# kimerein/sabatinilab-glm

Measured on AMD Instinct MI355X. Metric: IRLS iters/sec on 1M×2000 design mat; CV-grid wall-clock (5-fold×20 λ), lower is better.
Workload: dtype bf16 Hessian (w rounded to bf16, X exact 0/1) / exact-f32 gradient (3 bf16 pieces, f64 slab sums) / f64 coefficients and line search

## Files before the change

sabatinilab-glm_amd/csrc/chol.hip:

```cpp
#include <cstdlib>
#include <cstring>
#include <functional>
#include <map>
#include <mutex>
#include <vector>

#include "common.h"
#include "chol_tile.h"

namespace sglm {

constexpr int kNB = 64;
constexpr int kCT = 256;
constexpr int kMaxP = 8192;

void launch_chol_diag(int nact, hipStream_t s, float* Hall, int32_t P, int32_t k0,
                      const int32_t* fits, uint8_t* frozen_all, float* rhs_all,
                      const float* diag_all, int32_t* info, int32_t nrefac, float* minv_all,
                      float* Mall);
void launch_chol_diag4(int nact, hipStream_t s, float* Hall, int32_t P, int32_t k0,
                       const int32_t* fits, uint8_t* frozen_all, const float* diag_all,
                       int32_t* info, float* minv_all, float* Mall);

void launch_chol_diag4q(int nact, hipStream_t s, float* Hall, int32_t P, int32_t k0,
                        const int32_t* fits, uint8_t* frozen_all, const float* diag_all,
                        int32_t* info, float* minv_all, float* Mall);
void launch_chol_diag4l(int nact, hipStream_t s, float* Hall, int32_t P, int32_t k0,
                        const int32_t* fits, uint8_t* frozen_all, const float* diag_all,
                        int32_t* info, float* minv_all, float* Mall);
void launch_chol_update_diag4l(dim3 grid, hipStream_t s, float* Hall, int32_t P, int32_t k0,
                               int32_t kc, int32_t s0, const int32_t* fits, uint8_t* frozen_all,
                               const float* diag_all, int32_t* info, float* minv_all,
                               float* Mall);

static bool diag4q() {
    const char* e = getenv("SGLM_DIAG4Q");
    return !(e && e[0] == '0');
}

static bool diag4l() {
    const char* e = getenv("SGLM_DIAG4L");
    return !(e && e[0] == '0');
}

static bool upd_diag() {
    const char* e = getenv("SGLM_UPD_DIAG");
    return !(e && e[0] == '0');
}

static bool diag4() {
    static const bool v = [] {
        const char* e = getenv("SGLM_DIAG4");
        return !(e && e[0] == '0');
    }();
    return v;
}


__global__ void __launch_bounds__(kCT) chol_prep_kernel(
    float* __restrict__ Hall, int32_t P, const int32_t* __restrict__ fits,
    const double* __restrict__ gall, const float* __restrict__ dshift_all,
    uint8_t* __restrict__ frozen_all, float* __restrict__ rhs_all, float* __restrict__ diag_all,
    int32_t* __restrict__ info, int32_t nrefac) {
    const int fit = fits[blockIdx.x];
    const bool refactor = (int)blockIdx.x < nrefac;
    float* H = Hall + (int64_t)fit * P * P;
    const float* dsh = dshift_all + (int64_t)fit * P;
    uint8_t* frz = frozen_all + (int64_t)fit * P;
    float* rhs = rhs_all + (int64_t)fit * P;
    float* dg = diag_all + (int64_t)fit * P;
    const int tid = threadIdx.x;
    if (refactor) {
        if (tid == 0) info[fit] = 0;
        for (int j = tid; j < P; j += kCT) {
            const float d = H[(int64_t)j * P + j] + dsh[j];
            const bool f = dsh[j] < 0.0f || !(d > 0.0f);
            frz[j] = f;
            dg[j] = f ? 1.0f : d;
            H[(int64_t)j * P + j] = f ? 1.0f : d;
        }
    }
    if (!gall) return;
    const double* g = gall + (int64_t)fit * P;
    __syncthreads();
    for (int j = tid; j < P; j += kCT) rhs[j] = frz[j] ? 0.0f : (float)g[j];
}

__global__ void __launch_bounds__(kCT) chol_freeze_kernel(float* __restrict__ Hall, int32_t P,
                                                          const int32_t* __restrict__ fits,
                                                          const uint8_t* __restrict__ frozen_all) {
    const int fit = fits[blockIdx.y];
    float* H = Hall + (int64_t)fit * P * P;
    const uint8_t* frz = frozen_all + (int64_t)fit * P;
    int t = blockIdx.x, bi = 0;
    {
        int rowlen = P / kNB;
        while (t >= rowlen) { t -= rowlen; ++bi; --rowlen; }
    }
    const int bj = bi + t;
    __shared__ uint8_t fr[kNB], fc[kNB];
    __shared__ int any;
    const int tid = threadIdx.x;
    if (tid == 0) any = 0;
    __syncthreads();
    if (tid < kNB) {
        fr[tid] = frz[bi * kNB + tid];
        if (fr[tid]) any = 1;
    } else if (tid < 2 * kNB) {
        fc[tid - kNB] = frz[bj * kNB + tid - kNB];
        if (fc[tid - kNB]) any = 1;
    }
    __syncthreads();
    if (!any) return;
    const int c = tid & 63;
    for (int r = tid >> 6; r < kNB; r += kCT / 64) {
        const int i = bi * kNB + r, j = bj * kNB + c;
        if (i > j || !(fr[r] | fc[c])) continue;
        H[(int64_t)i * P + j] = i == j ? 1.0f : 0.0f;
    }
}

__global__ void __launch_bounds__(kCT) chol_alias_prep_kernel(
    int32_t P, const int32_t* __restrict__ fits, const int32_t* __restrict__ fsrc,
    const double* __restrict__ gall, const float* __restrict__ rscale,
    const uint8_t* __restrict__ frozen_all, float* __restrict__ rhs_all) {
    const int fit = fits[blockIdx.x];
    const uint8_t* frz = frozen_all + (int64_t)fsrc[blockIdx.x] * P;
    const double* g = gall + (int64_t)fit * P;
    float* rhs = rhs_all + (int64_t)fit * P;
    const double sc = (double)rscale[blockIdx.x];
    for (int j = threadIdx.x; j < P; j += kCT) rhs[j] = frz[j] ? 0.0f : (float)(g[j] * sc);
}

__device__ __forceinline__ float lanef(float v, int l) {
    return __int_as_float(__builtin_amdgcn_readlane(__float_as_int(v), l));
}

__global__ void __launch_bounds__(kCT) chol_panel_kernel(
    float* __restrict__ Hall, int32_t P, int32_t k0, const int32_t* __restrict__ fits,
    const float* __restrict__ minv_all, float* __restrict__ rhs_all, int32_t nrefac) {
    __shared__ float zs[kNB];
    __shared__ float sred[2][kNB];
    const int slot = blockIdx.x;
    const int fit = fits[slot];
    const bool refactor = slot < nrefac;
    float* H = Hall + (int64_t)fit * P * P;
    float* rhs = rhs_all + (int64_t)fit * P;
    const int tid = threadIdx.x, lane = tid & 63, wave = tid >> 6;
    const int r32 = lane & 31, kh = lane >> 5;
    const int rh = wave >> 1, ch = wave & 1;
    const int j0 = k0 + kNB + blockIdx.y * kNB;
    const int j = j0 + ch * 32 + r32;
    if (tid < kNB) zs[tid] = rhs[k0 + tid];
    float b[32];
    const float* pb = H + (int64_t)(k0 + kh) * P + j;
#pragma unroll
    for (int u = 0; u < 32; ++u) b[u] = pb[(int64_t)(2 * u) * P];
    __syncthreads();
    float s = 0.0f;
    if (refactor) {
        const float* pm = minv_all + (int64_t)slot * kNB * kNB + (rh * 32 + r32) * kNB + kh;
        float m[32];
#pragma unroll
        for (int u = 0; u < 32; ++u) m[u] = (rh || u < 16) ? pm[2 * u] : 0.0f;
        f32x16 acc = {};
#pragma unroll
        for (int u = 0; u < 16; ++u)
            acc = __builtin_amdgcn_mfma_f32_32x32x2f32(m[u], b[u], acc, 0, 0, 0);
        if (rh) {
#pragma unroll
            for (int u = 16; u < 32; ++u)
                acc = __builtin_amdgcn_mfma_f32_32x32x2f32(m[u], b[u], acc, 0, 0, 0);
        }
        __syncthreads();
#pragma unroll
        for (int q = 0; q < 16; ++q) {
            const int i = rh * 32 + (q & 3) + 8 * (q >> 2) + 4 * kh;
            H[(int64_t)(k0 + i) * P + j] = acc[q];
            s = fmaf(acc[q], zs[i], s);
        }
    } else if (rh == 0) {
#pragma unroll
        for (int u = 0; u < 32; ++u) s = fmaf(b[u], zs[2 * u + kh], s);
    }
    s += __shfl_xor(s, 32, 64);
    if (kh == 0) sred[rh][ch * 32 + r32] = s;
// ... 673 lines not shown
            for (int u = 0; u < 4; ++u) {
                float b[2];
#pragma unroll
                for (int qj = 0; qj < 2; ++qj)
                    b[qj] = sb[cur][(4 * kh + 8 * kk + u) * kLB2 + wc * 64 + qj * 32 + r32];
#pragma unroll
                for (int qi = 0; qi < 2; ++qi)
#pragma unroll
                    for (int qj = 0; qj < 2; ++qj)
                        acc[qi][qj] = __builtin_amdgcn_mfma_f32_32x32x2f32(a[qi][u], b[qj],
                                                                           acc[qi][qj], 0, 0, 0);
            }
        }
        if (more) sstore(cur ^ 1);
        __syncthreads();
        cur ^= 1;
    }
#pragma unroll
    for (int qi = 0; qi < 2; ++qi)
#pragma unroll
        for (int qj = 0; qj < 2; ++qj) {
            const int i0 = ti * kT2 + wr * 64 + qi * 32, j0 = tj * kT2 + wc * 64 + qj * 32;
#pragma unroll
            for (int q = 0; q < 16; ++q) {
                const int i = i0 + (q & 3) + 8 * (q >> 2) + 4 * kh, j = j0 + r32;
                if (STEP == 0)
                    T[(int64_t)i * s + j] = acc[qi][qj][q];
                else
                    M[(int64_t)(a0 + i) * P + c0 + j] = -acc[qi][qj][q];
            }
        }
}

template <bool SECOND, bool STAGE = false>
__global__ void __launch_bounds__(kCT) chol_inv_apply_kernel(
    const float* __restrict__ Mall, int32_t P, const int32_t* __restrict__ fits,
    const int32_t* __restrict__ fsrc, const float* __restrict__ rscale,
    const int32_t* __restrict__ tiles, const double* __restrict__ gall,
    const uint8_t* __restrict__ frozen_all, float* __restrict__ Y, float* __restrict__ delta_all) {
    __shared__ float red[4][16 * 64];
    __shared__ __attribute__((aligned(16))) float sm[STAGE ? 4 : 1][STAGE ? 64 * 32 : 4];
    const int start = tiles[2 * blockIdx.y], cnt = tiles[2 * blockIdx.y + 1];
    const int src = fsrc[start];
    const float* M = Mall + (int64_t)src * P * P;
    const uint8_t* frz = frozen_all + (int64_t)src * P;
    const int lane = threadIdx.x & 63, wave = threadIdx.x >> 6;
    const int r32 = lane & 31, kh = lane >> 5;
    const int c0 = blockIdx.x * 32;
    const bool valid = r32 < cnt;
    const int q = start + (valid ? r32 : 0);
    f32x16 acc = {};
    if (!SECOND) {
        const double* g = gall + (int64_t)fits[q] * P;
        const double sc = (double)rscale[q];
        const float* pb = M + c0 + r32;
        const int khi = (c0 / kNB + 1) * kNB;
        for (int kb = kNB * wave; kb < khi; kb += 4 * kNB) {
            float a[8][4], b[8][4];
            const float* pbk = pb + (int64_t)(kb + 4 * kh) * P;
            if (STAGE) {
                const float* src = M + (int64_t)kb * P + c0 + 4 * (lane & 7);
                f32x4 tv[8];
#pragma unroll
                for (int i = 0; i < 8; ++i)
                    tv[i] = *reinterpret_cast<const f32x4*>(src + (int64_t)((lane >> 3) + 8 * i) * P);
#pragma unroll
                for (int i = 0; i < 8; ++i)
                    *reinterpret_cast<f32x4*>(&sm[wave][((lane >> 3) + 8 * i) * 32 + 4 * (lane & 7)]) =
                        tv[i];
                asm volatile("s_waitcnt lgkmcnt(0)" ::: "memory");
                __builtin_amdgcn_wave_barrier();
            }
#pragma unroll
            for (int v = 0; v < 8; ++v) {
                const int k = kb + 8 * v + 4 * kh;
                const uint32_t fz = *reinterpret_cast<const uint32_t*>(frz + k);
                const double2 g01 = *reinterpret_cast<const double2*>(g + k);
                const double2 g23 = *reinterpret_cast<const double2*>(g + k + 2);
                a[v][0] = (float)(g01.x * sc);
                a[v][1] = (float)(g01.y * sc);
                a[v][2] = (float)(g23.x * sc);
                a[v][3] = (float)(g23.y * sc);
                const uint32_t keep = valid ? ~fz : 0u;
#pragma unroll
                for (int u = 0; u < 4; ++u) {
                    if (((keep >> (8 * u)) & 0xff) != 0xff) a[v][u] = 0.0f;
                    b[v][u] = STAGE ? sm[wave][(8 * v + 4 * kh + u) * 32 + r32]
                                    : pbk[(8 * v + u) * P];
                }
            }
#pragma unroll
            for (int v = 0; v < 8; ++v)
#pragma unroll
                for (int u = 0; u < 4; ++u)
                    acc = __builtin_amdgcn_mfma_f32_32x32x2f32(a[v][u], b[v][u], acc, 0, 0, 0);
            if (STAGE) {
                asm volatile("s_waitcnt lgkmcnt(0)" ::: "memory");
                __builtin_amdgcn_wave_barrier();
            }
        }
    } else {
        const float* py = Y + (int64_t)q * P;
        const float* pm = M + (int64_t)(c0 + r32) * P;
        const int klo = (c0 / kNB) * kNB;
        for (int kb = klo + kNB * wave; kb < P; kb += 4 * kNB) {
            f32x4 a[8], b[8];
#pragma unroll
            for (int v = 0; v < 8; ++v) {
                const int k = kb + 8 * v + 4 * kh;
                a[v] = *reinterpret_cast<const f32x4*>(py + k);
                if (!valid) a[v] = f32x4{0.0f, 0.0f, 0.0f, 0.0f};
                b[v] = *reinterpret_cast<const f32x4*>(pm + k);
            }
#pragma unroll
            for (int v = 0; v < 8; ++v)
#pragma unroll
                for (int u = 0; u < 4; ++u)
                    acc = __builtin_amdgcn_mfma_f32_32x32x2f32(a[v][u], b[v][u], acc, 0, 0, 0);
        }
    }
#pragma unroll
    for (int r = 0; r < 16; ++r) red[wave][r * 64 + lane] = acc[r];
    __syncthreads();
#pragma unroll
    for (int m = 0; m < 4; ++m) {
        const int o = threadIdx.x + kCT * m;
        const float v = red[0][o] + red[1][o] + red[2][o] + red[3][o];
        const int r = o >> 6, l = o & 63;
        const int row = (r & 3) + 8 * (r >> 2) + 4 * (l >> 5), col = c0 + (l & 31);
        if (row >= cnt) continue;
        if (!SECOND)
            Y[(int64_t)(start + row) * P + col] = v;
        else
            delta_all[(int64_t)fits[start + row] * P + col] = frz[col] ? 0.0f : -v;
    }
}

}

using namespace sglm;

static int64_t inv_tcap(int32_t P) {
    int64_t cap = 0;
    for (int s = kNB; s < P; s *= 2) {
        const int64_t pairs = (P - s + 2 * s - 1) / (2 * s);
        const int64_t v = pairs * s * s;
        cap = v > cap ? v : cap;
    }
    return cap;
}

extern "C" size_t sglm_chol_work_bytes(int32_t P, int32_t B) {
    return ((size_t)3 * (size_t)B * (size_t)P + (size_t)B * kNB * kNB +
            (size_t)B * (size_t)inv_tcap(P)) * sizeof(float);
}

static int chol_lookahead() {
    const char* e = getenv("SGLM_CHOL_LOOKAHEAD");
    const int v = e ? atoi(e) : 4;
    return v >= 1 && v <= 8 ? v : 4;
}

static bool inv_pipe() {
    static const bool v = [] {
        const char* e = getenv("SGLM_CHOL_PIPE");
        return !(e && e[0] == '0');
    }();
    return v;
}

static bool inv_x3() {
    const char* e = getenv("SGLM_INV_X3");
    return !(e && e[0] == '0');
}

static bool inv_lds() {
    static const bool v = [] {
        const char* e = getenv("SGLM_INV_LDS");
        return !(e && e[0] == '0');
    }();
    return v;
}

static bool inv128(int64_t wgs) {
    const char* e = getenv("SGLM_INV128_WG");
    const int64_t mn = e ? atoll(e) : 0;
    return mn > 0 && wgs >= mn;
}

static bool upd_pipe() {
    static const bool v = [] {
        const char* e = getenv("SGLM_UPD_PIPE");
        return e && e[0] == '1';
    }();
    return v;
}

static bool apply_stage() {
    static const bool v = [] {
        const char* e = getenv("SGLM_APPLY_STAGE");
        return !(e && e[0] == '0');
    }();
    return v;
}

static bool upd_lds() {
    static const bool v = [] {
        const char* e = getenv("SGLM_UPD_LDS");
        return !(e && e[0] == '0');
    }();
    return v;
}

static void launch_update(dim3 grid, hipStream_t s, float* H, int32_t P, int32_t k0, int32_t kc,
                          int32_t s0, const int32_t* fits) {
    if (upd_lds())
        chol_update_lds_kernel<<<grid, kCT, 0, s>>>(H, P, k0, kc, s0, fits);
    else if (upd_pipe())
        chol_update_kernel<true><<<grid, kCT, 0, s>>>(H, P, k0, kc, s0, fits);
    else
        chol_update_kernel<false><<<grid, kCT, 0, s>>>(H, P, k0, kc, s0, fits);
}

static int chol_solve_mixed(float* H, int32_t P, const int32_t* fits, int32_t nact,
                            int32_t nrefac, const double* g, const float* dshift, float* delta,
                            int32_t* info, uint8_t* frozen, int32_t B, void* work,
                            hipStream_t s, float* Mall = nullptr,
                            const std::function<void(int)>* on_diag = nullptr) {
    if (nact <= 0) return SGLM_OK;
    if (!H || !fits || (!g && !Mall) || !dshift || !delta || !info || !frozen || !work ||
        P % kNB || P > kMaxP || B < nact || nrefac < 0 || nrefac > nact) {
        set_error("sglm_chol_solve: bad args (P=%d, max %d)", P, kMaxP);
        return SGLM_EINVAL;
    }
    float* rhs = (float*)work;
    float* dg = rhs + (size_t)B * P;
    float* minv = dg + (size_t)B * P;
    chol_prep_kernel<<<nact, kCT, 0, s>>>(H, P, fits, g, dshift, frozen, rhs, dg, info, nrefac);
    int st = check_launch("chol_prep_kernel");
    if (st) return st;
    if (nrefac > 0) {
        const int nb = P / kNB;
        chol_freeze_kernel<<<dim3((unsigned)(nb * (nb + 1) / 2), (unsigned)nrefac), kCT, 0, s>>>(
            H, P, fits, frozen);
        if ((st = check_launch("chol_freeze_kernel"))) return st;
    }
    if (nrefac == 0 && Mall) return SGLM_OK;
    if (nrefac == 0) {
        chol_fwd2_kernel<<<nact, kST, 0, s>>>(H, P, fits, nullptr, frozen, rhs);
        st = check_launch("chol_fwd2_kernel");
        if (st) return st;
        chol_back2_kernel<<<nact, kST, 0, s>>>(H, P, fits, nullptr, frozen, rhs, delta);
        return check_launch("chol_back2_kernel");
    }
    const int nb = P / kNB;
    const bool fuse = Mall && nrefac == nact && diag4() && diag4q() && diag4l() && upd_lds() &&
                      upd_diag();
    bool have_diag = false;
    auto factor_step = [&](int kb) {
        const int k0 = kb * kNB;
        if (have_diag)
            ;
        else if (Mall && nrefac == nact && diag4() && diag4q() && diag4l())
            launch_chol_diag4l(nact, s, H, P, k0, fits, frozen, dg, info, minv, Mall);
        else if (Mall && nrefac == nact && diag4() && diag4q())
            launch_chol_diag4q(nact, s, H, P, k0, fits, frozen, dg, info, minv, Mall);
        else if (Mall && nrefac == nact && diag4())
            launch_chol_diag4(nact, s, H, P, k0, fits, frozen, dg, info, minv, Mall);
        else
            launch_chol_diag(nact, s, H, P, k0, fits, frozen, rhs, dg, info, nrefac, minv, Mall);
        if (!have_diag && on_diag) (*on_diag)(kb);
        const int rem = P - k0 - kNB;
        if (rem > 0)
            chol_panel_kernel<<<dim3(nact, rem / kNB), kCT, 0, s>>>(H, P, k0, fits, minv, rhs,
                                                                    nrefac);
    };
    const int la = chol_lookahead();
    for (int kb = 0; kb < nb; kb += la) {
        const int ke = kb + la < nb ? kb + la : nb;
        for (int b = kb; b < ke; ++b) {
            factor_step(b);
            have_diag = false;
            const int nr = ke - 1 - b;
            const int T = nb - b - 1;
            if (nrefac > 0 && nr > 0) {
                const dim3 g(nr * T - nr * (nr - 1) / 2, nrefac);
                if (fuse) {
                    launch_chol_update_diag4l(g, s, H, P, b * kNB, kNB, b + 1, fits, frozen, dg,
                                              info, minv, Mall);
                    have_diag = true;
                    if (on_diag) (*on_diag)(b + 1);
                } else {
                    launch_update(g, s, H, P, b * kNB, kNB, b + 1, fits);
                }
            }
        }
        const int T = nb - ke;
        if (nrefac > 0 && T > 0) {
            const dim3 g(T * (T + 1) / 2, nrefac);
            if (fuse) {
                launch_chol_update_diag4l(g, s, H, P, kb * kNB, (ke - kb) * kNB, ke, fits, frozen,
                                          dg, info, minv, Mall);
                have_diag = true;
                if (on_diag) (*on_diag)(ke);
            } else {
                launch_update(g, s, H, P, kb * kNB, (ke - kb) * kNB, ke, fits);
            }
        }
    }
    st = check_launch("chol block kernels");
    if (st) return st;
    if (Mall) return SGLM_OK;
    chol_back2_kernel<<<nact, kST, 0, s>>>(H, P, fits, nullptr, frozen, rhs, delta);
    return check_launch("chol_back2_kernel");
}

extern "C" int sglm_chol_solve_ex(float* H, int32_t P, const int32_t* fits, int32_t nact,
                                  const double* g, const float* dshift, float* delta,
                                  int32_t* info, uint8_t* frozen, int32_t refactor,
                                  int32_t B, void* work, sglm_stream_t stream) {
    return chol_solve_mixed(H, P, fits, nact, refactor ? nact : 0, g, dshift, delta, info,
                            frozen, B, work, as_stream(stream));
}

extern "C" int sglm_chol_solve_alias(const float* H, int32_t P, const int32_t* fits,
                                     const int32_t* fsrc, int32_t nact, const double* g,
                                     const float* rscale, float* delta, const uint8_t* frozen,
                                     int32_t B, void* work, sglm_stream_t stream) {
    if (nact <= 0) return SGLM_OK;
    if (!H || !fits || !fsrc || !g || !rscale || !delta || !frozen || !work || P % kNB ||
        P > kMaxP || B < nact) {
        set_error("sglm_chol_solve_alias: bad args (P=%d)", P);
        return SGLM_EINVAL;
    }
    hipStream_t s = as_stream(stream);
    float* rhs = (float*)work;
    chol_alias_prep_kernel<<<nact, kCT, 0, s>>>(P, fits, fsrc, g, rscale, frozen, rhs);
    int st = check_launch("chol_alias_prep_kernel");
    if (st) return st;
    chol_fwd2_kernel<<<nact, kST, 0, s>>>(H, P, fits, fsrc, frozen, rhs);
    st = check_launch("chol_fwd2_kernel");
    if (st) return st;
    chol_back2_kernel<<<nact, kST, 0, s>>>(H, P, fits, fsrc, frozen, rhs, delta);
    return check_launch("chol_back2_kernel");
}

extern "C" int sglm_chol_solve_mixed(float* H, int32_t P, const int32_t* fits, int32_t nact,
                                     int32_t nrefac, const double* g, const float* dshift,
                                     float* delta, int32_t* info, uint8_t* frozen, int32_t B,
                                     void* work, sglm_stream_t stream) {
    return chol_solve_mixed(H, P, fits, nact, nrefac, g, dshift, delta, info, frozen, B, work,
                            as_stream(stream));
}


static bool inv_col() {
// ... 125 lines not shown
int chain_cache_cap() {
    static const int cap = [] {
        const char* e = getenv("SGLM_CHOL_GRAPH_CAP");
        const int v = e ? atoi(e) : 32;
        return v > 0 ? v : 1;
    }();
    return cap;
}

void chain_entry_destroy(ChainEntry& e) {
    if (e.done) {
        (void)hipEventSynchronize(e.done);
        (void)hipEventDestroy(e.done);
    }
    if (e.exec) (void)hipGraphExecDestroy(e.exec);
    e.exec = nullptr;
    e.done = nullptr;
}

void chain_cache_evict_to(size_t keep) {
    while (g_chain_cache.size() > keep) {
        auto lru = g_chain_cache.begin();
        for (auto it = g_chain_cache.begin(); it != g_chain_cache.end(); ++it)
            if (it->second.used < lru->second.used) lru = it;
        g_chain_pending.push_back(lru->second);
        g_chain_cache.erase(lru);
    }
}

void chain_pending_reap(bool wait) {
    std::vector<ChainEntry> done;
    {
        std::lock_guard<std::mutex> lock(g_chain_mu);
        for (size_t i = 0; i < g_chain_pending.size();) {
            ChainEntry& e = g_chain_pending[i];
            if (wait || !e.done || hipEventQuery(e.done) == hipSuccess) {
                done.push_back(e);
                e = g_chain_pending.back();
                g_chain_pending.pop_back();
            } else {
                ++i;
            }
        }
    }
    for (auto& e : done) chain_entry_destroy(e);
}
}

extern "C" int32_t sglm_chol_graph_cache_size(void) {
    std::lock_guard<std::mutex> lock(g_chain_mu);
    return (int32_t)g_chain_cache.size();
}

extern "C" int sglm_chol_graph_cache_clear(void) {
    {
        std::lock_guard<std::mutex> lock(g_chain_mu);
        chain_cache_evict_to(0);
    }
    chain_pending_reap(true);
    return SGLM_OK;
}

static int factor_inv_cached(float* H, float* Minv, int32_t P, const int32_t* fits, int32_t n,
                             const float* dshift, float* delta, int32_t* info, uint8_t* frozen,
                             int32_t B, void* work, hipStream_t s, InvColCtx* ctx, bool levels);

static int factor_inv(float* H, float* Minv, int32_t P, const int32_t* fits, int32_t n,
                      const float* dshift, float* delta, int32_t* info, uint8_t* frozen,
                      int32_t B, void* work, hipStream_t s, bool levels = true) {
    InvColCtx* ctx = (levels && inv_col()) ? inv_col_ctx(P / kNB + 1) : nullptr;
    if (!chol_graphs_enabled() || s == nullptr)
        return factor_inv_launch(H, Minv, P, fits, n, dshift, delta, info, frozen, B, work, s,
                                 ctx, levels);
    const int st = factor_inv_cached(H, Minv, P, fits, n, dshift, delta, info, frozen, B, work, s,
                                     ctx, levels);
    chain_pending_reap(false);
    return st;
}

static int factor_inv_cached(float* H, float* Minv, int32_t P, const int32_t* fits, int32_t n,
                             const float* dshift, float* delta, int32_t* info, uint8_t* frozen,
                             int32_t B, void* work, hipStream_t s, InvColCtx* ctx, bool levels) {
    ChainKey key;
    std::memset(&key, 0, sizeof(key));
    key.H = H; key.Minv = Minv; key.fits = fits; key.dshift = dshift; key.delta = delta;
    key.info = info; key.frozen = frozen; key.work = work;
    key.P = P; key.n = n; key.B = B; key.la = chol_lookahead(); key.q = (diag4q() ? (diag4l() ? (upd_diag() ? 3 : 2) : 1) : 0) | (ctx ? 4 : 0) | (levels ? 0 : 8) | (inv_x3() ? 16 : 0);
    std::lock_guard<std::mutex> lock(g_chain_mu);
    auto it = g_chain_cache.find(key);
    if (it == g_chain_cache.end()) {
        hipGraph_t graph = nullptr;
        if (hipStreamBeginCapture(s, hipStreamCaptureModeThreadLocal) != hipSuccess) {
            set_error("chol graph: hipStreamBeginCapture failed");
            return SGLM_EHIP;
        }
        const int st = factor_inv_launch(H, Minv, P, fits, n, dshift, delta, info, frozen, B,
                                         work, s, ctx, levels);
        const hipError_t ec = hipStreamEndCapture(s, &graph);
        if (st) {
            if (graph) (void)hipGraphDestroy(graph);
            return st;
        }
        if (ec != hipSuccess || !graph) {
            set_error("chol graph: hipStreamEndCapture failed");
            return SGLM_EHIP;
        }
        ChainEntry e;
        const hipError_t ei = hipGraphInstantiate(&e.exec, graph, nullptr, nullptr, 0);
        (void)hipGraphDestroy(graph);
        if (ei != hipSuccess) {
            set_error("chol graph: hipGraphInstantiate failed");
            return SGLM_EHIP;
        }
        if (hipEventCreateWithFlags(&e.done, hipEventDisableTiming) != hipSuccess) {
            (void)hipGraphExecDestroy(e.exec);
            set_error("chol graph: hipEventCreate failed");
            return SGLM_EHIP;
        }
        chain_cache_evict_to((size_t)chain_cache_cap() - 1);
        it = g_chain_cache.emplace(key, e).first;
    }
    it->second.used = ++g_chain_tick;
    if (hipGraphLaunch(it->second.exec, s) != hipSuccess) {
        set_error("chol graph: hipGraphLaunch failed");
        return SGLM_EHIP;
    }
    if (hipEventRecord(it->second.done, s) != hipSuccess) {
        set_error("chol graph: hipEventRecord failed");
        return SGLM_EHIP;
    }
    return SGLM_OK;
}

extern "C" int sglm_chol_solve_inv(float* H, float* Minv, int32_t P, const int32_t* fits,
                                   const int32_t* fsrc, const float* rscale, int32_t nact,
                                   int32_t nrefac, const int32_t* tiles, int32_t ntiles,
                                   const double* g, const float* dshift, float* delta,
                                   int32_t* info, uint8_t* frozen, int32_t B, void* work,
                                   sglm_stream_t stream) {
    if (nact <= 0) return SGLM_OK;
    if (!H || !Minv || !fits || (ntiles > 0 && (!fsrc || !rscale || !tiles || !g)) || !delta ||
        !frozen || !work || P % kNB || P > kMaxP || B < nact || nrefac < 0 || nrefac > nact ||
        (nrefac > 0 && (!dshift || !info))) {
        set_error("sglm_chol_solve_inv: bad args (P=%d, max %d)", P, kMaxP);
        return SGLM_EINVAL;
    }
    hipStream_t s = as_stream(stream);
    int st;
    if (nrefac > 0 && (st = factor_inv(H, Minv, P, fits, nrefac, dshift, delta, info, frozen, B,
                                       work, s)))
        return st;
    if (ntiles <= 0) return SGLM_OK;
    float* Y = (float*)work + (size_t)2 * B * P + (size_t)B * kNB * kNB;
    const dim3 grid((unsigned)(P / 32), (unsigned)ntiles);
    if (apply_stage())
        chol_inv_apply_kernel<false, true><<<grid, kCT, 0, s>>>(Minv, P, fits, fsrc, rscale, tiles,
                                                               g, frozen, Y, delta);
    else
        chol_inv_apply_kernel<false><<<grid, kCT, 0, s>>>(Minv, P, fits, fsrc, rscale, tiles, g,
                                                           frozen, Y, delta);
    chol_inv_apply_kernel<true><<<grid, kCT, 0, s>>>(Minv, P, fits, fsrc, rscale, tiles, g,
                                                      frozen, Y, delta);
    return check_launch("chol_inv_apply_kernel");
}

extern "C" int sglm_chol_factor(float* H, float* Minv, int32_t P, const int32_t* fits,
                                int32_t n, const float* dshift, int32_t* info, uint8_t* frozen,
                                int32_t B, void* work, sglm_stream_t stream) {
    if (n <= 0) return SGLM_OK;
    if (!H || !Minv || !fits || !dshift || !info || !frozen || !work || P % kNB || P > kMaxP ||
        B < n) {
        set_error("sglm_chol_factor: bad args (P=%d, max %d)", P, kMaxP);
        return SGLM_EINVAL;
    }
    float* scratch = (float*)work + (size_t)2 * B * P + (size_t)B * kNB * kNB;
    return factor_inv(H, Minv, P, fits, n, dshift, scratch, info, frozen, B, work,
                      as_stream(stream), false);
}

extern "C" int sglm_chol_invert(const float* H, float* Minv, int32_t P, const int32_t* fits,
                                int32_t n, int32_t B, void* work, sglm_stream_t stream) {
    if (n <= 0) return SGLM_OK;
    if (!H || !Minv || !fits || !work || P % kNB || P > kMaxP || B < n) {
        set_error("sglm_chol_invert: bad args (P=%d, max %d)", P, kMaxP);
        return SGLM_EINVAL;
    }
    return inv_levels(H, Minv, P, fits, n, B, work, as_stream(stream));
}
```

sabatinilab-glm_amd/sglm_hip/engine.py:

```python
from __future__ import annotations

import ctypes
import math
import os
import threading
import types
from dataclasses import dataclass, field
from typing import List, Optional, Sequence

import numpy as np

from . import _lib

try:
    import torch
except ImportError as e:
    raise _lib.HipEngineUnavailable("PyTorch-ROCm is required for device memory") from e

FAM_SQUARED = 0
FAM_TWEEDIE_LOG = 1
X_BF16, X_F32 = 0, 1
COL_PAD = 256
ROW_PAD = 256
ARMIJO_SIGMA = 2.0 ** -11
# ... 1656 lines not shown
                grad_d, grad_n, grad_bp = carried
                carried = None
            else:
                grad_d, grad_n, grad_bp = act_d, na, pad_to(na, 32)
        g_copy = None
        link_d, link_n = act_d, na
        if GRAD_DEDUP and use_rp and fused and not dev_linked and linked is None:
            own_ok = drift[act] <= reuse_tol
            is_cand = (repl[act] >= 0) & ~no_alias[act] & ~own_ok
            lead_of, first = {}, {}
            for k in act[~is_cand & ~own_ok]:
                if fresh_start[k]:
                    first.setdefault(hkey(k), int(k))
            for k in act:
                if fresh_start[k]:
                    rk = first.setdefault(hkey(k), int(k))
                    if rk != k:
                        lead_of[int(k)] = rk
            if lead_of:
                lead = np.array([k for k in act if int(k) not in lead_of], dtype=np.int32)
                link_d, link_n = up(lead, np.int32), int(lead.size)
                grad_d, grad_n, grad_bp = link_d, link_n, pad_to(link_n, 32)
                cp = up(np.array([[k, r] for k, r in lead_of.items()], np.int64).T.reshape(-1),
                        np.int64)
                g_copy = (cp[:len(lead_of)], cp[len(lead_of):])
                if stats is not None:
                    stats.grad_dedup += len(lead_of)
        if fused and not dev_linked:
            if linked is None:
                _lib.call("sglm_link_update", fam, power, n, ld, link_n, _p(link_d), _p(bf.eta),
                          _p(prob.Y), _p(prob.M), _p(fit_resp), _p(fit_mask), None, R_out,
                          Rp_out, None, None, st)
        else:
            _lib.call("sglm_link_update", fam, power, n, ld, B, None, _p(bf.eta), _p(prob.Y),
                      _p(prob.M), _p(fit_resp), _p(fit_mask), None, _p(bf.R), None, None,
                      None, st)

        grad_done = [False]

        def _gradient(cochain_ok=True):
            if grad_done[0]:
                return
            grad_done[0] = True
            if use_lag:
                lg = d.lag
                _lib.call("sglm_lag_xtr", _p(lg.occ), _p(lg.tbeg), _p(lg.tend), _p(lg.shifts),
                          lg.m, lg.K, lg.layout, lg.row0, n, P, _p(bf.R), ld, _p(act_d), na,
                          _p(bf.g), _p(lag_work), st)
            elif use_rp:
                cochain = (cochain_ok and XTR_COCHAIN and nref > 0 and SOLVE_INV
                           and CHOL_STREAM != "serial")
                if ev_px is not None and (XTR_EVENTS == "1" or xtr_events_auto(grad_n)):
                    lg = d.lag
                    _lib.call("sglm_lag_xtr_packed_bp", _p(lg.occ), int(lg.occ.numel()),
                              _p(ev_px[0]), _p(ev_px[1]), lg.m, lg.K, lg.smin, lg.smax,
                              lg.layout, lg.row0, n, ld, P, _p(rp_buf), grad_n, grad_bp,
                              _p(grad_d), _p(bf.g), _p(ev_work),
                              XTR_EVENTS_COWG if cochain else 2, st)
                    if stats is not None:
                        stats.grad_events += 1
                else:
                    if cochain:
                        _lib.call("sglm_xtr_prefer", 1)
                    try:
                        _lib.call("sglm_xtr_bits_packed_bp", _p(d.cbits_full()), ld, P, n,
                                  _p(rp_buf), grad_n, grad_bp, _p(grad_d), _p(bf.g),
                                  _p(gx_work), st)
                    finally:
                        if cochain:
                            _lib.call("sglm_xtr_prefer", -1)
                d.mix_xtr(2, rp_buf, ld, grad_bp, None, grad_d, grad_n, bf.g)
                if g_copy is not None:
                    bf.g[g_copy[0]] = bf.g[g_copy[1]]
            else:
                d.xtr(bf.R, B, bf.g)
            if comm is not None:
                comm.sum_(bf.g[:B])
            torch.addcmul(bf.g[:B], lamp_d, beta64_d[:B], out=bf.gtot[:B])

        if pending_inv is not None:
            torch.cuda.current_stream().wait_event(pending_inv)
            pending_inv = None
        gram_comp = np.zeros(B, dtype=bool)
        pipe_groups = None
        if const_hess:
            gram_now[:] = not factored
            if not factored:
                reps = {}
                for k in act:
                    reps.setdefault(reqs[k].mask, k)
                rep_idx = np.array(sorted(reps.values()), dtype=np.int32)
                _link_weights(bf, rep_idx, st)
                _syrk(d, bf, rep_idx, nsteps, ntile1, stats, st, exact=True, rows=gram_rows)
                sum_hess(rep_idx)
                gram_comp[rep_idx] = True
                f64 = _Factor64(d, bf, np.asarray([reps[reqs[k].mask] for k in k_d]),
                                np.asarray(k_d), lamp_d, st)
        else:
            if plan is None:
                plan = hess_plan(act)
            if GRAD_FIRST and plan["form"].size == 0 and plan["npairs"] and SOLVE_INV:
                _gradient(cochain_ok=False)
            keep, form, uniq, dup, ali, fail, exact_h = hess_finish(plan)
            plan = None
            alias[:] = -1
            alias[ali] = repl[ali]
            pipe_groups = _gram_groups(form, uniq, dup) if (
                GRAM_PIPE > 0 and SOLVE_INV and CHOL_STREAM != "serial" and comm is None) else None
            if pipe_groups is None:
                lagg = np.array([k for k in uniq if fresh_start[k] and all_rows[k]],
                                dtype=np.int32) if use_lag_gram else np.zeros(0, np.int32)
                if lagg.size:
                    _lag_gram(d, bf, lagg, st)
                    if stats is not None:
                        stats.lag_grams += int(lagg.size)
                        stats.alg_flop += _lag_corr_flop(d.lag)
                _syrk(d, bf, np.sort(np.setdiff1d(uniq, lagg)).astype(np.int32), nsteps,
                      ntile1, stats, st, rows=gram_rows)
                sum_hess(uniq)
                for k, rk in dup:
                    bf.H[k].copy_(bf.H[rk])
            else:
                form = np.concatenate([g for _, g in pipe_groups]).astype(form.dtype)
            gram_comp[uniq] = True
            gram_now[:] = False
            gram_now[form] = True
            if stats is not None:
                stats.gram_fits += int(uniq.size)
                stats.reused += int(keep.size)
                stats.aliased += int(ali.size)
                stats.shared += int(np.sum(~exact_h[form]))
        t0 = tick("it_gram", t0)
        bf.delta[:B].zero_()
        if const_hess:
            order, nref = act, 0
            _gradient()
            t0 = tick("it_gradient", t0)
            _lib.call("sglm_chol64_solve", _p(f64.U), P, _p(f64.state), _p(act_d),
                      _p(fkey_d[act_d.long()]), na, _p(bf.gtot), _p(bf.delta), st)
        elif SOLVE_INV:
            order, nref = np.concatenate([form, keep]), form.size
            al = ali[np.argsort(repl[ali], kind="stable")] if (not const_hess and ali.size) \
                else np.zeros(0, dtype=np.int64)
            src = repl[al]
            if dist_f:
                fowner[order[:nref]] = comm.owners(int(nref), rot)
                rot += int(nref)
                mine_f = fowner == comm.rank
                fo, ko = order[:nref], order[nref:]
                fo, ko = fo[mine_f[fo]], ko[mine_f[ko]]
                order, nref = np.concatenate([fo, ko]), int(fo.size)
                sel = mine_f[src]
                al, src = al[sel], src[sel]
            lst = np.concatenate([order, al]).astype(np.int32)
            fsrc = np.concatenate([order, src]).astype(np.int32)
            rsc = np.concatenate([np.ones(order.size), rows[src] / rows[al]]).astype(np.float32)
            tiles = [(q, 1) for q in range(order.size)]
            q = order.size
            while q < lst.size:
                e = q
                while e < lst.size and e - q < 32 and fsrc[e] == fsrc[q]:
                    e += 1
                tiles.append((q, e - q))
                q = e
            ints = up(np.concatenate([lst, fsrc, np.asarray(tiles, np.int32).reshape(-1)]),
                      np.int32)
            rsc_d = up(rsc, np.float32)
            nl = int(lst.size)
            fact_done = None
            defer = False
            if pending_inv is not None:
                torch.cuda.current_stream().wait_event(pending_inv)
                pending_inv = None
            if nref and CHOL_STREAM == "serial":
                bf.fact_fits[:nref].copy_(ints[:nref])
                _lib.call("sglm_chol_solve_inv", _p(bf.H), _p(bf.Minv), P, _p(bf.fact_fits), None,
                          None, int(nref), int(nref), None, 0, None, _p(bf.dshift), _p(bf.delta),
                          _p(bf.info), _p(bf.frozen), B, _p(bf.cwork), st)
            elif nref:
                side = _side_stream()
                bf.fact_fits[:nref].copy_(ints[:nref])
                chains = []
                if pipe_groups is not None:
                    off = 0
                    dsrc = dict(dup)
                    if GRAM_PIPE == 1:
                        batches = [[g] for g in pipe_groups]
                    else:
                        h = (len(pipe_groups) + 1) // 2
                        batches = [pipe_groups[:h], pipe_groups[h:]]
                    for bt in batches:
                        srcs = np.array(sorted(int(r) for r, _ in bt), dtype=np.int32)
                        _syrk(d, bf, srcs, nsteps, ntile1, stats, st, rows=gram_rows)
                        nb_ = 0
                        for r, grp in bt:
                            for k in grp:
                                if int(k) != int(r):
                                    bf.H[int(k)].copy_(bf.H[int(dsrc[int(k)])])
                            nb_ += int(len(grp))
                        ready = torch.cuda.Event()
                        ready.record()
                        chains.append((ready, off, nb_))
                        off += nb_
                else:
                    ready = torch.cuda.Event()
                    ready.record()
                    nsplit = CHOL_SPLIT if nref >= CHOL_SPLIT_MIN else 1
                    cuts = np.linspace(0, int(nref), nsplit + 1).round().astype(int)
                    chains += [(ready, int(cuts[j]), int(cuts[j + 1] - cuts[j]))
                               for j in range(nsplit) if cuts[j + 1] > cuts[j]]
                    defer = (DEFER_INV_MIN > 0 and nref >= DEFER_INV_MIN and len(chains) == 1
                             and comm is None)
                _gradient()
                t0 = tick("it_gradient", t0)
                dones = []
                for j, (ready, off, ng) in enumerate(chains):
                    sd = side if (pipe_groups is not None or j == 0) else _side_stream(j)
                    sd.wait_event(ready)
                    t_ch = time.perf_counter()
                    if defer:
                        _lib.call("sglm_chol_factor", _p(bf.H), _p(bf.Minv), P,
                                  _p(bf.fact_fits[off:]), ng, _p(bf.dshift), _p(bf.info),
                                  _p(bf.frozen), B, _p(bf.chol_work(0)), sd.cuda_stream)
                    else:
                        _lib.call("sglm_chol_solve_inv", _p(bf.H), _p(bf.Minv), P,
                                  _p(bf.fact_fits[off:]), None, None, ng, ng, None, 0, None,
                                  _p(bf.dshift), _p(bf.delta), _p(bf.info), _p(bf.frozen), B,
                                  _p(bf.chol_work(j if pipe_groups is None else 0)),
                                  sd.cuda_stream)
                    if stats is not None:
                        stats.chain_host_s += time.perf_counter() - t_ch
                    if sd is not side:
                        ev_ = torch.cuda.Event()
                        ev_.record(sd)
                        dones.append(ev_)
                for ev_ in dones:
                    side.wait_event(ev_)
                fact_done = torch.cuda.Event()
                fact_done.record(side)
                if defer:
                    _lib.call("sglm_chol_invert", _p(bf.H), _p(bf.Minv), P, _p(bf.fact_fits),
                              int(nref), B, _p(bf.chol_work(0)), side.cuda_stream)
                    pending_inv = torch.cuda.Event()
                    pending_inv.record(side)
            if fact_done is None:
                _gradient()
                t0 = tick("it_gradient", t0)
            if fact_done is not None:
                torch.cuda.current_stream().wait_event(fact_done)
            if nl and defer:
                newf = np.isin(fsrc, order[:nref])
                if (~newf).any():
                    lo, fo, ro = lst[~newf], fsrc[~newf], rsc[~newf]
                    tl, q = [], 0
                    while q < lo.size:
                        e = q + 1
                        while e < lo.size and e - q < 32 and fo[e] == fo[q]:
                            e += 1
                        tl.append((q, e - q))
                        q = e
                    io = up(np.concatenate([lo, fo, np.asarray(tl, np.int32).reshape(-1)]),
                            np.int32)
                    no = int(lo.size)
                    _lib.call("sglm_chol_solve_inv", _p(bf.H), _p(bf.Minv), P, _p(io),
                              _p(io[no:]), _p(up(ro, np.float32)), no, 0, _p(io[2 * no:]),
                              len(tl), _p(bf.gtot), _p(bf.dshift), _p(bf.delta), _p(bf.info),
                              _p(bf.frozen), B, _p(bf.cwork), st)
                ln, fn, rn = lst[newf], fsrc[newf], rsc[newf]
                idn = up(np.stack([ln, fn]), np.int32)
                _lib.call("sglm_chol_solve_alias", _p(bf.H), P, _p(idn[0]), _p(idn[1]),
                          int(ln.size), _p(bf.gtot), _p(up(rn, np.float32)), _p(bf.delta),
                          _p(bf.frozen), B, _p(bf.cwork), st)
            elif nl:
                _lib.call("sglm_chol_solve_inv", _p(bf.H), _p(bf.Minv), P, _p(ints),
                          _p(ints[nl:]), _p(rsc_d), nl, 0, _p(ints[2 * nl:]), len(tiles),
                          _p(bf.gtot), _p(bf.dshift), _p(bf.delta), _p(bf.info), _p(bf.frozen),
                          B, _p(bf.cwork), st)
            if comm is not None and (dist_f or not comm.distribute):
                owned = np.zeros(B0, dtype=np.uint8)
                owned[lst] = 1
                comm.directions_(bf.delta[:B], up(owned, np.uint8))
        else:
            order, nref = np.concatenate([form, keep]), form.size
            _gradient()
            t0 = tick("it_gradient", t0)
            fits_d = up(order, np.int32)
            _lib.call("sglm_chol_solve_mixed", _p(bf.H), P, _p(fits_d), int(order.size),
                      int(nref), _p(bf.gtot), _p(bf.dshift), _p(bf.delta), _p(bf.info),
                      _p(bf.frozen), B, _p(bf.cwork), st)
        if not SOLVE_INV and not const_hess and ali.size:
            src = repl[ali]
            al_d = up(np.stack([ali, src]), np.int32)
            rscale_d = up(rows[src] / rows[ali], np.float32)
            _lib.call("sglm_chol_solve_alias", _p(bf.H), P, _p(al_d[0]), _p(al_d[1]),
                      int(ali.size), _p(bf.gtot), _p(rscale_d), _p(bf.delta), _p(bf.frozen), B,
                      _p(bf.cwork), st)
        factored = True
        aa_idx = None
        if use_aa:
            fepoch[form] += 1
            src_now = np.where(alias[act] >= 0, alias[act], act)
            key_now = src_now * 1_000_000 + fepoch[src_now]
            aa_idx = up(act, np.int64)
            selm = (aa_key[act] == key_now) & ~gram_now[act] & (aa_t[act] > 0)
            sel = np.flatnonzero(selm)
            if AA_KERNEL:
                _lib.call("sglm_aa_step", P, p, na, _p(act_d), _p(up(selm.astype(np.uint8))),
                          _p(up(aa_t[act], np.float32)), _p(bf.delta), _p(aa_raw), _p(aa_used),
                          _p(bf.gtot), _p(aa_rm), st)
                if stats is not None:
                    stats.aa_fit_iters += int(sel.size)
                sel = sel[:0]
            else:
                raw = bf.delta[aa_idx]
                aa_rm.zero_()
            if sel.size:
                sel_d = up(sel, np.int64)
                f = raw[sel_d]
                df = f - aa_raw[aa_idx[sel_d]]
                db = aa_used[aa_idx[sel_d]] * up(aa_t[act[sel]], np.float32)[:, None]
                den = (df * df).sum(1)
                gam = (df * f).sum(1) / den.clamp_min(1e-30)
                dnew = f - gam[:, None] * (db + df)
                gdn = (bf.gtot[aa_idx[sel_d]].float() * dnew).sum(1)
                good = (den > 1e-12 * (f * f).sum(1)) & (gam >= -2.0) & (gam <= 0.5) & (gdn < 0)
                bf.delta[aa_idx[sel_d]] = torch.where(good[:, None], dnew, f)
                aa_rm[aa_idx[sel_d], 0] = f[:, :p].abs().amax(1)
                aa_rm[aa_idx[sel_d], 1] = f[:, p].abs()
                if stats is not None:
                    stats.aa_fit_iters += int(sel.size)
            if not AA_KERNEL:
                aa_raw[aa_idx] = raw
            aa_key[act] = key_now
        d.eta(bf.delta, bf.deta, slots=act_d, direction=True)
# ... 1243 lines not shown
```

Baseline: 0.02566.

## Add streaming two-pass inverse-apply kernels and group aliases with their source fits

Adds a new opt-in path, enabled by SGLM_APPLY_STREAM=1, that computes delta = -Minv*g as a streaming two-stage product. Each stage writes partial sums per row block or column chunk, and separate reduction kernels sum them, which costs extra workspace. Host-side tiling now groups each factored fit together with the aliased fits that share its inverse, so tiles span more right-hand sides per Minv read. The factored-fit list is passed separately because lst no longer starts with the factor order. The new kernel is off by default, but the regrouped tiles affect the default apply path too.

Result: no change. 0.02531 (median of 5 runs) (-1.4%).

```diff
diff --git a/sabatinilab-glm_amd/csrc/chol.hip b/sabatinilab-glm_amd/csrc/chol.hip
--- a/sabatinilab-glm_amd/csrc/chol.hip
+++ b/sabatinilab-glm_amd/csrc/chol.hip
@@ -32,6 +32,12 @@
                                int32_t kc, int32_t s0, const int32_t* fits, uint8_t* frozen_all,
                                const float* diag_all, int32_t* info, float* minv_all,
                                float* Mall);
+
+size_t inv_stream_work_floats(int32_t P, int32_t B);
+int launch_inv_apply_stream(hipStream_t s, const float* Minv, int32_t P, const int32_t* fits,
+                            const int32_t* fsrc, const float* rscale, const int32_t* tiles,
+                            int32_t ntiles, const double* g, const uint8_t* frozen, int32_t B,
+                            float* Y, float* part, float* delta);
 
 static bool diag4q() {
     const char* e = getenv("SGLM_DIAG4Q");
@@ -1011,7 +1017,7 @@
 
 extern "C" size_t sglm_chol_work_bytes(int32_t P, int32_t B) {
     return ((size_t)3 * (size_t)B * (size_t)P + (size_t)B * kNB * kNB +
-            (size_t)B * (size_t)inv_tcap(P)) * sizeof(float);
+            (size_t)B * (size_t)inv_tcap(P) + inv_stream_work_floats(P, B)) * sizeof(float);
 }
 
 static int chol_lookahead() {
@@ -1061,6 +1067,11 @@
         return !(e && e[0] == '0');
     }();
     return v;
+}
+
+static bool apply_stream() {
+    const char* e = getenv("SGLM_APPLY_STREAM");
+    return e && e[0] == '1';
 }
 
 static bool upd_lds() {
@@ -1492,6 +1503,11 @@
         return st;
     if (ntiles <= 0) return SGLM_OK;
     float* Y = (float*)work + (size_t)2 * B * P + (size_t)B * kNB * kNB;
+    if (apply_stream())
+        return launch_inv_apply_stream(
+            s, Minv, P, fits, fsrc, rscale, tiles, ntiles, g, frozen, B, Y,
+            (float*)work + (size_t)3 * B * P + (size_t)B * kNB * kNB + (size_t)B * inv_tcap(P),
+            delta);
     const dim3 grid((unsigned)(P / 32), (unsigned)ntiles);
     if (apply_stage())
         chol_inv_apply_kernel<false, true><<<grid, kCT, 0, s>>>(Minv, P, fits, fsrc, rscale, tiles,
diff --git a/sabatinilab-glm_amd/csrc/chol_apply.hip b/sabatinilab-glm_amd/csrc/chol_apply.hip
--- /dev/null
+++ b/sabatinilab-glm_amd/csrc/chol_apply.hip
@@ -0,0 +1,277 @@
+#include "common.h"
+
+namespace sglm {
+
+namespace {
+
+constexpr int kCT = 256;
+constexpr int kAQ = 8;
+constexpr int kAK = 128;
+constexpr int kAJ = 256;
+constexpr int kAR = 64;
+constexpr int kGS = kAQ + 4;
+
+template <int N>
+__device__ __forceinline__ void pair_sum(const float* v, float* w, int mask, bool odd) {
+#pragma unroll
+    for (int t = 0; t < N / 2; ++t) {
+        const float a = v[2 * t], b = v[2 * t + 1];
+        const float got = __shfl_xor(odd ? a : b, mask, 64);
+        w[t] = (odd ? b : a) + got;
+    }
+}
+
+__device__ __forceinline__ f32x4 ldm(uint64_t sbase, uint32_t voff) {
+    f32x4 v;
+    asm volatile("global_load_dwordx4 %0, %1, %2" : "=v"(v) : "v"(voff), "s"(sbase) : "memory");
+    return v;
+}
+
+template <int NB>
+__device__ __forceinline__ void y_item(float* gs, uint64_t sb, uint32_t voff, uint64_t rstep,
+                                       int P, int k0, int kend, int start, int cnt,
+                                       const int32_t* __restrict__ fits,
+                                       const float* __restrict__ rscale,
+                                       const double* __restrict__ gall,
+                                       const uint8_t* __restrict__ frz, float* yo) {
+    const int lane = threadIdx.x & 63, rg = lane >> 4;
+    const int k = threadIdx.x & (kAK - 1), kk = k0 + k, kc = min(kk, kend - 1);
+    for (int q0 = 0; q0 < cnt; q0 += kAQ) {
+        f32x4 mb[2][8];
+        if constexpr (NB > 0) {
+#pragma unroll
+            for (int h = 0; h < 2; ++h)
+#pragma unroll
+                for (int i = 0; i < 8; ++i) mb[h][i] = ldm(sb + (uint64_t)(8 * h + i) * rstep, voff);
+        }
+        if (q0) __syncthreads();
+        {
+            constexpr int kIt = kAK * kAQ / kCT;
+            const bool kz = kk >= kend || frz[kc] != 0;
+            int fit[kIt];
+            float sc[kIt];
+            double gv[kIt];
+#pragma unroll
+            for (int it = 0; it < kIt; ++it) {
+                const int qq = min(q0 + 2 * it + (int)(threadIdx.x >> 7), cnt - 1);
+                fit[it] = fits[start + qq];
+                sc[it] = rscale[start + qq];
+            }
+#pragma unroll
+            for (int it = 0; it < kIt; ++it) gv[it] = gall[(int64_t)fit[it] * P + kc];
+#pragma unroll
+            for (int it = 0; it < kIt; ++it) {
+                const int q = 2 * it + (int)(threadIdx.x >> 7);
+                const float v = (float)(gv[it] * (double)sc[it]);
+                gs[k * kGS + q] = (kz || q0 + q >= cnt) ? 0.0f : v;
+            }
+        }
+        __syncthreads();
+        if constexpr (NB > 0) {
+            float acc[4 * kAQ];
+#pragma unroll
+            for (int t = 0; t < 4 * kAQ; ++t) acc[t] = 0.0f;
+#pragma unroll
+            for (int b = 0; b < NB; ++b) {
+                if (b + 1 < NB)
+                    asm volatile("s_waitcnt vmcnt(8)" ::: "memory");
+                else
+                    asm volatile("s_waitcnt vmcnt(0)" ::: "memory");
+#pragma unroll
+                for (int i = 0; i < 8; ++i) asm volatile("" : "+v"(mb[b & 1][i]));
+#pragma unroll
+                for (int i = 0; i < 8; ++i) {
+                    const float* gp = &gs[(32 * b + 4 * i + rg) * kGS];
+                    const f32x4 g0 = *reinterpret_cast<const f32x4*>(gp);
+                    const f32x4 g1 = *reinterpret_cast<const f32x4*>(gp + 4);
+                    const f32x4 m = mb[b & 1][i];
+#pragma unroll
+                    for (int q = 0; q < kAQ; ++q) {
+                        const float gq = q < 4 ? g0[q & 3] : g1[q & 3];
+#pragma unroll
+                        for (int c = 0; c < 4; ++c)
+                            acc[4 * q + c] = __builtin_fmaf(gq, m[c], acc[4 * q + c]);
+                    }
+                }
+                if (b + 2 < NB) {
+#pragma unroll
+                    for (int t = 0; t < 4 * kAQ; ++t) asm volatile("" : "+v"(acc[t]));
+#pragma unroll
+                    for (int i = 0; i < 8; ++i)
+                        mb[b & 1][i] = ldm(sb + (uint64_t)(8 * (b + 2) + i) * rstep, voff);
+                }
+            }
+            float w1[2 * kAQ], w2[kAQ];
+            pair_sum<4 * kAQ>(acc, w1, 16, rg & 1);
+            pair_sum<2 * kAQ>(w1, w2, 32, rg >> 1);
+#pragma unroll
+            for (int q = 0; q < kAQ; ++q)
+                if (q0 + q < cnt) yo[(int64_t)(q0 + q) * P] = w2[q];
+        }
+    }
+}
+
+__global__ void __launch_bounds__(kCT) inv_stream_y_kernel(
+    const float* __restrict__ Mall, int32_t P, const int32_t* __restrict__ fits,
+    const int32_t* __restrict__ fsrc, const float* __restrict__ rscale,
+    const int32_t* __restrict__ tiles, const double* __restrict__ gall,
+    const uint8_t* __restrict__ frozen_all, float* __restrict__ Yp, int64_t cs) {
+    __shared__ __attribute__((aligned(16))) float gs[kAK * kGS];
+    const int nseg = (P + kAJ - 1) / kAJ;
+    const int r = blockIdx.x / nseg, sg = blockIdx.x % nseg;
+    const int k0 = r * kAK;
+    if ((sg + 1) * kAJ <= k0) return;
+    const int start = tiles[2 * blockIdx.y], cnt = tiles[2 * blockIdx.y + 1];
+    const int src = fsrc[start];
+    const float* M = Mall + (int64_t)src * P * P;
+    const uint8_t* frz = frozen_all + (int64_t)src * P;
+    const int lane = threadIdx.x & 63;
+    const int wave = __builtin_amdgcn_readfirstlane((int)(threadIdx.x >> 6));
+    const int rg = lane >> 4, c4 = lane & 15;
+    const int c0 = sg * kAJ + wave * 64;
+    const int kend = min(k0 + kAK, P);
+    const bool live = c0 < P && c0 >= k0;
+    const int nb = live ? (min(kend, c0 + 64) - k0) / 32 : 0;
+    const uint64_t sb = (uint64_t)(M + (int64_t)k0 * P + (live ? c0 : 0));
+    const uint32_t voff = (uint32_t)(rg * P + 4 * c4) * 4u;
+    const uint64_t rstep = (uint64_t)P * 16u;
+    float* yo = Yp + (int64_t)r * cs + (int64_t)start * P + c0 + 4 * c4 + rg;
+    if (nb == 4)
+        y_item<4>(gs, sb, voff, rstep, P, k0, kend, start, cnt, fits, rscale, gall, frz, yo);
+    else if (nb == 2)
+        y_item<2>(gs, sb, voff, rstep, P, k0, kend, start, cnt, fits, rscale, gall, frz, yo);
+    else
+        y_item<0>(gs, sb, voff, rstep, P, k0, kend, start, cnt, fits, rscale, gall, frz, yo);
+}
+
+__global__ void __launch_bounds__(kCT) inv_stream_ysum_kernel(
+    const float* __restrict__ Yp, int64_t cs, int32_t P, const int32_t* __restrict__ tiles,
+    float* __restrict__ Y) {
+    const int j = ((int)blockIdx.x * kCT + (int)threadIdx.x) * 4;
+    if ((int)blockIdx.y >= tiles[2 * blockIdx.z + 1] || j >= P) return;
+    const int64_t e = (int64_t)(tiles[2 * blockIdx.z] + (int)blockIdx.y) * P + j;
+    f32x4 s = *reinterpret_cast<const f32x4*>(Yp + e);
+    for (int r = 1; r <= j / kAK; ++r) s += *reinterpret_cast<const f32x4*>(Yp + r * cs + e);
+    *reinterpret_cast<f32x4*>(Y + e) = s;
+}
+
+__global__ void __launch_bounds__(kCT, 4) inv_stream_d_kernel(
+    const float* __restrict__ Mall, int32_t P, const int32_t* __restrict__ fsrc,
+    const int32_t* __restrict__ tiles, const float* __restrict__ Y, float* __restrict__ Dp,
+    int64_t cs) {
+    __shared__ __attribute__((aligned(16))) float ys[kAQ * kAJ];
+    const int nch = (P + kAJ - 1) / kAJ;
+    const int i0 = (blockIdx.x / nch) * kAR, ch = blockIdx.x % nch;
+    const int jc0 = ch * kAJ;
+    if (jc0 + kAJ <= i0) return;
+    const int start = tiles[2 * blockIdx.y], cnt = tiles[2 * blockIdx.y + 1];
+    const float* M = Mall + (int64_t)fsrc[start] * P * P;
+    const int lane = threadIdx.x & 63;
+    const int wave = __builtin_amdgcn_readfirstlane((int)(threadIdx.x >> 6));
+    const int rg = lane >> 4, c4 = lane & 15;
+    const int iw = i0 + 16 * wave;
+    const uint64_t sb = (uint64_t)(M + (int64_t)iw * P + jc0);
+    const uint32_t voff = (uint32_t)(rg * P + 4 * c4) * 4u;
+    const uint64_t rstep = (uint64_t)P * 16u;
+    const int plo = max(0, (i0 - jc0) / 64);
+    f32x4 m[4][4];
+#pragma unroll
+    for (int p = 0; p < 4; ++p) {
+        const int jp = jc0 + 64 * p;
+        const int pe = (jp >= i0 && jp < P) ? p : plo;
+#pragma unroll
+        for (int l = 0; l < 4; ++l) m[p][l] = ldm(sb + (uint64_t)pe * 256u + (uint64_t)l * rstep, voff);
+    }
+    const int j = jc0 + (int)threadIdx.x, jc = min(j, P - 1);
+    for (int q0 = 0; q0 < cnt; q0 += kAQ) {
+        if (q0) __syncthreads();
+        {
+            float yv[kAQ];
+#pragma unroll
+            for (int q = 0; q < kAQ; ++q)
+                yv[q] = Y[(int64_t)(start + min(q0 + q, cnt - 1)) * P + jc];
+#pragma unroll
+            for (int q = 0; q < kAQ; ++q)
+                ys[q * kAJ + threadIdx.x] = (q0 + q < cnt && j < P) ? yv[q] : 0.0f;
+        }
+        __syncthreads();
+        asm volatile("s_waitcnt vmcnt(0)" ::: "memory");
+#pragma unroll
+        for (int p = 0; p < 4; ++p)
+#pragma unroll
+            for (int l = 0; l < 4; ++l) asm volatile("" : "+v"(m[p][l]));
+        float acc[4 * kAQ];
+#pragma unroll
+        for (int t = 0; t < 4 * kAQ; ++t) acc[t] = 0.0f;
+#pragma unroll
+        for (int p = 0; p < 4; ++p) {
+            const int jp = jc0 + 64 * p;
+            if (jp >= i0 && jp < P) {
+#pragma unroll
+                for (int q = 0; q < kAQ; ++q) {
+                    const f32x4 yv = *reinterpret_cast<const f32x4*>(&ys[q * kAJ + 64 * p + 4 * c4]);
+#pragma unroll
+                    for (int l = 0; l < 4; ++l)
+#pragma unroll
+                        for (int c = 0; c < 4; ++c)
+                            acc[kAQ * l + q] = __builtin_fmaf(m[p][l][c], yv[c], acc[kAQ * l + q]);
+                }
+            }
+        }
+        float w1[16], w2[8], w3[4], w4[2];
+        pair_sum<32>(acc, w1, 1, c4 & 1);
+        pair_sum<16>(w1, w2, 2, (c4 >> 1) & 1);
+        pair_sum<8>(w2, w3, 4, (c4 >> 2) & 1);
+        pair_sum<4>(w3, w4, 8, (c4 >> 3) & 1);
+        const int q = c4 & 7;
+        if (q0 + q < cnt) {
+            float* po = Dp + (int64_t)ch * cs + (int64_t)(start + q0 + q) * P + iw + rg;
+#pragma unroll
+            for (int t = 0; t < 2; ++t) po[4 * (2 * t + (c4 >> 3))] = w4[t];
+        }
+    }
+}
+
+__global__ void __launch_bounds__(kCT) inv_stream_dsum_kernel(
+    const float* __restrict__ Dp, int64_t cs, int32_t P, const int32_t* __restrict__ tiles,
+    const int32_t* __restrict__ fits, const int32_t* __restrict__ fsrc,
+    const uint8_t* __restrict__ frozen_all, float* __restrict__ delta_all) {
+    const int i = ((int)blockIdx.x * kCT + (int)threadIdx.x) * 4;
+    if ((int)blockIdx.y >= tiles[2 * blockIdx.z + 1] || i >= P) return;
+    const int q = tiles[2 * blockIdx.z] + (int)blockIdx.y;
+    const int64_t e = (int64_t)q * P + i;
+    const int nch = (P + kAJ - 1) / kAJ;
+    const int c0 = i / kAJ;
+    f32x4 s = *reinterpret_cast<const f32x4*>(Dp + c0 * cs + e);
+    for (int c = c0 + 1; c < nch; ++c) s += *reinterpret_cast<const f32x4*>(Dp + c * cs + e);
+    const uint8_t* frz = frozen_all + (int64_t)fsrc[q] * P + i;
+    f32x4 o;
+#pragma unroll
+    for (int u = 0; u < 4; ++u) o[u] = frz[u] ? 0.0f : -s[u];
+    *reinterpret_cast<f32x4*>(delta_all + (int64_t)fits[q] * P + i) = o;
+}
+
+}
+
+size_t inv_stream_work_floats(int32_t P, int32_t B) {
+    return (size_t)((P + kAK - 1) / kAK + (P + kAJ - 1) / kAJ) * (size_t)B * (size_t)P;
+}
+
+int launch_inv_apply_stream(hipStream_t s, const float* Minv, int32_t P, const int32_t* fits,
+                            const int32_t* fsrc, const float* rscale, const int32_t* tiles, int32_t ntiles, const double* g,
+                            const uint8_t* frozen, int32_t B, float* Y, float* part,
+                            float* delta) {
+    const int n1 = (P + kAK - 1) / kAK, nj = (P + kAJ - 1) / kAJ;
+    const int64_t cs = (int64_t)B * P;
+    float* Dp = part + (size_t)n1 * cs;
+    const dim3 gsum((unsigned)((P / 4 + kCT - 1) / kCT), 32u, (unsigned)ntiles);
+    inv_stream_y_kernel<<<dim3((unsigned)(n1 * nj), (unsigned)ntiles), kCT, 0, s>>>(
+        Minv, P, fits, fsrc, rscale, tiles, g, frozen, n1 > 1 ? part : Y, cs);
+    if (n1 > 1) inv_stream_ysum_kernel<<<gsum, kCT, 0, s>>>(part, cs, P, tiles, Y);
+    inv_stream_d_kernel<<<dim3((unsigned)((P / kAR) * nj), (unsigned)ntiles), kCT, 0, s>>>(
+        Minv, P, fsrc, tiles, Y, Dp, cs);
+    inv_stream_dsum_kernel<<<gsum, kCT, 0, s>>>(Dp, cs, P, tiles, fits, fsrc, frozen, delta);
+    return check_launch("inv_stream_apply");
+}
+
+}
diff --git a/sabatinilab-glm_amd/sglm_hip/engine.py b/sabatinilab-glm_amd/sglm_hip/engine.py
--- a/sabatinilab-glm_amd/sglm_hip/engine.py
+++ b/sabatinilab-glm_amd/sglm_hip/engine.py
@@ -1832,19 +1832,22 @@
                 order, nref = np.concatenate([fo, ko]), int(fo.size)
                 sel = mine_f[src]
                 al, src = al[sel], src[sel]
-            lst = np.concatenate([order, al]).astype(np.int32)
-            fsrc = np.concatenate([order, src]).astype(np.int32)
-            rsc = np.concatenate([np.ones(order.size), rows[src] / rows[al]]).astype(np.float32)
-            tiles = [(q, 1) for q in range(order.size)]
-            q = order.size
-            while q < lst.size:
-                e = q
-                while e < lst.size and e - q < 32 and fsrc[e] == fsrc[q]:
-                    e += 1
-                tiles.append((q, e - q))
-                q = e
-            ints = up(np.concatenate([lst, fsrc, np.asarray(tiles, np.int32).reshape(-1)]),
-                      np.int32)
+            al_by = {}
+            for a_, s_ in zip(al.tolist(), src.tolist()):
+                al_by.setdefault(s_, []).append(a_)
+            runs = [(int(f), [int(f)] + al_by.pop(int(f), [])) for f in order]
+            runs += list(al_by.items())
+            lst = np.asarray([k for _, ks in runs for k in ks], dtype=np.int32)
+            fsrc = np.asarray([f for f, ks in runs for _ in ks], dtype=np.int32)
+            rsc = (rows[fsrc] / rows[lst]).astype(np.float32)
+            tiles, q = [], 0
+            for _, ks in runs:
+                for o in range(0, len(ks), 32):
+                    tiles.append((q + o, min(32, len(ks) - o)))
+                q += len(ks)
+            ints = up(np.concatenate([lst, fsrc, np.asarray(tiles, np.int32).reshape(-1),
+                                      order[:nref].astype(np.int32)]), np.int32)
+            fact_src = ints[ints.numel() - int(nref):]
             rsc_d = up(rsc, np.float32)
             nl = int(lst.size)
             fact_done = None
@@ -1853,13 +1856,13 @@
                 torch.cuda.current_stream().wait_event(pending_inv)
                 pending_inv = None
             if nref and CHOL_STREAM == "serial":
-                bf.fact_fits[:nref].copy_(ints[:nref])
+                bf.fact_fits[:nref].copy_(fact_src)
                 _lib.call("sglm_chol_solve_inv", _p(bf.H), _p(bf.Minv), P, _p(bf.fact_fits), None,
                           None, int(nref), int(nref), None, 0, None, _p(bf.dshift), _p(bf.delta),
                           _p(bf.info), _p(bf.frozen), B, _p(bf.cwork), st)
             elif nref:
                 side = _side_stream()
-                bf.fact_fits[:nref].copy_(ints[:nref])
+                bf.fact_fits[:nref].copy_(fact_src)
                 chains = []
                 if pipe_groups is not None:
                     off = 0
```
